# DerrickXuNu/CoBEVT

Measured on AMD Instinct MI355X. Metric: bev_frames_per_sec, higher is better.
Workload: dtype bf16

## Files before the change

cobevt_amd/csrc/basicblock.hip:

```cpp
#include "common.hpp"

namespace cobevt {

struct BasicBlockParams {
    const void* in;
    const uint4* w1;
    const float* b1;
    const uint4* w2;
    const float* b2;
    void* out;
    int N, H, W;
    int tiles_y, tiles_x;
    int ntiles;
};

#ifndef COBEVT_BB_PERSIST
#define COBEVT_BB_PERSIST 1
#endif

template <typename T, int C, int TH_> struct BBCfg {
    static constexpr int NT = 512;
    static constexpr int EB = Elem<T>::kBytes, CH = Elem<T>::kChunk;
    static constexpr int CC = 128 / EB;
    static constexpr int NCH = C / CC;
    static constexpr int NCT = C / 32;
    static constexpr int NPG = 8 / NCT;
    static constexpr int TH = TH_, TW = 16;
    static constexpr int R1H = TH + 2, R1W = TW + 2, R1 = R1H * R1W;
    static constexpr int N1 = (R1 + 31) / 32;
// ... 69 lines not shown
                    __builtin_amdgcn_sched_group_barrier(0x008, 1, 0);
                }
            }
            __builtin_amdgcn_sched_barrier(0);
        }
    }
}

#ifdef COBEVT_BB_TRACE
__device__ unsigned long long cobevt_bb_trace[32];
#define COBEVT_BB_MARK(i) do { if (blockIdx.x == 0 && threadIdx.x == 0) cobevt_bb_trace[(i)] = __builtin_readcyclecounter(); } while (0)
#else
#define COBEVT_BB_MARK(i) do {} while (0)
#endif

template <typename T, int C, int TH_>
__global__ __launch_bounds__(512, (C == 64 && TH_ == 8 && Elem<T>::kIsBf16) ? 4 : (TH_ == 12 ? 1 : 2)) void basicblock_kernel(BasicBlockParams p) {
    using G = BBCfg<T, C, TH_>;
    constexpr int NT = G::NT, CH = G::CH, CC = G::CC, NCH = G::NCH, NCT = G::NCT, NPG = G::NPG;
    constexpr int TH = G::TH, TW = G::TW, R1W = G::R1W, R1 = G::R1, N1 = G::N1, T1W = G::T1W, T2W = G::T2W;
    constexpr int P1W = G::P1W, PSTR1 = G::PSTR1, PSTR2 = G::PSTR2;
    constexpr int PIECES = 8;
    constexpr int P1_ITEMS = G::P1H * P1W * PIECES;
    constexpr int P_IT = (P1_ITEMS + NT - 1) / NT;
    constexpr int NSTEP = NCH * 9;
    constexpr int R = 3;

    extern __shared__ __attribute__((aligned(16))) unsigned char smem[];
    unsigned char* patch1 = smem;
    unsigned char* patch2 = smem + G::PATCH1;

    int logical;
// ... 135 lines not shown
                unsigned char* d = patch2 + ry * G::PITCH2 + rx * PSTR2 + (c0 + 8 * k) * Elem<T>::kBytes;
                if constexpr (Elem<T>::kIsBf16) *(uint2*)d = make_uint2(pack_bf2(v[0], v[1]), pack_bf2(v[2], v[3]));
                else if constexpr (kXPack<T, 4>)
                    *(uint2*)(patch2 + ry * G::PITCH2 + rx * PSTR2 + ct * 128 + packed_piece_offset(2 * k + h)) = make_uint2(pack_h2(v[0], v[1]), pack_h2(v[2], v[3]));
                else if constexpr (kXPack3<T, 4>)
                    store_piece_packed3(patch2 + ry * G::PITCH2 + rx * PSTR2 + ct * 128 + packed3_piece_offset(2 * k + h),
                                        make_uint4(__float_as_uint(v[0]), __float_as_uint(v[1]), __float_as_uint(v[2]), __float_as_uint(v[3])), false);
                else *(uint4*)d = stage_x_piece<T>(make_uint4(__float_as_uint(v[0]), __float_as_uint(v[1]), __float_as_uint(v[2]), __float_as_uint(v[3])));
            }
        }
    }
    constexpr int CPP = C / CH;
    constexpr int S_ITEMS = TH * TW * CPP;
    constexpr int S_IT = S_ITEMS / NT;
    static_assert(S_ITEMS % NT == 0, "store pass");
    int soff[S_IT];
    uint4 rres[S_IT];
#pragma unroll
    for (int i = 0; i < S_IT; ++i) {
        const int item = tid + i * NT;
        const int px = item / CPP, cj = item - px * CPP;
        const int oy = oy0 + px / TW, ox = ox0 + (px % TW);
        const bool ok = (oy < p.H) & (ox < p.W);
        soff[i] = ok ? ((img * p.H + oy) * p.W + ox) * C + cj * CH : -1;
        rres[i] = *(const uint4*)(in + (ok ? soff[i] : 0));
    }
    __builtin_amdgcn_sched_barrier(0);
    COBEVT_BB_MARK(8);
    __syncthreads();
    COBEVT_BB_MARK(9);

    f32x16 acc[T2W];
#pragma unroll
    for (int t = 0; t < T2W; ++t)
#pragma unroll
        for (int r = 0; r < 16; ++r) acc[t][r] = 0.f;
#pragma unroll 1
    for (int chunk = 0; chunk < NCH; ++chunk)
        bb_conv_chunk<T, T2W>(patch2 + chunk * 128, a2, t2_ok, G::PITCH2, PSTR2, w2src, chunk * 9, NSTEP, bq, acc);
    COBEVT_BB_MARK(10);
    const int next = tile + (int)gridDim.x;
    const bool has_next = G::PERSIST && next < p.ntiles;
    if (has_next) {
        set_tile(next);
        patch_addr();
        load_patch(0);
    }
    __syncthreads();
    COBEVT_BB_MARK(11);

    float* stage = (float*)smem;
    constexpr int SROW = G::SSTR / 4;
    {
        const int c0 = ct * 32 + 4 * h;
#pragma unroll
        for (int t = 0; t < T2W; ++t) {
            const int px = (pg + t * NPG) * 32 + ql;
#pragma unroll
            for (int k = 0; k < 4; ++k) {
                const float4 b = *(const float4*)&sbias[C + c0 + 8 * k];
                *(float4*)(stage + px * SROW + c0 + 8 * k) =
                    make_float4(acc[t][4 * k] + b.x, acc[t][4 * k + 1] + b.y, acc[t][4 * k + 2] + b.z, acc[t][4 * k + 3] + b.w);
            }
        }
    }
    __syncthreads();
    COBEVT_BB_MARK(12);
    T* out = (T*)p.out;
    float sv[S_IT][CH];
#pragma unroll
    for (int i = 0; i < S_IT; ++i) {
        const int item = tid + i * NT;
        const int px = item / CPP, cj = item - px * CPP;
#pragma unroll
        for (int e = 0; e < CH; ++e) sv[i][e] = stage[px * SROW + cj * CH + e];
    }
    if (has_next) __syncthreads();
#pragma unroll
    for (int i = 0; i < S_IT; ++i) {
        if (soff[i] < 0) continue;
        float v[8], rv[8];
#pragma unroll
        for (int e = 0; e < CH; ++e) v[e] = sv[i][e];
        chunk_to_f32<T>(rres[i], rv);
#pragma unroll
        for (int e = 0; e < CH; ++e) v[e] = fmaxf(v[e] + rv[e], 0.f);
        *(uint4*)(out + soff[i]) = f32_to_chunk<T>(v);
    }
    COBEVT_BB_MARK(13);
    if (!has_next) break;
    tile = next;
    load_b(bq[0], w1src, 0);
    load_b(bq[1], w1src, 1);
  }
}

template <typename T, int C, int TH_>
static int launch_basicblock(BasicBlockParams p, hipStream_t stream) {
    using G = BBCfg<T, C, TH_>;
    p.tiles_y = (p.H + G::TH - 1) / G::TH;
    p.tiles_x = (p.W + G::TW - 1) / G::TW;
    long blocks = (long)p.N * p.tiles_y * p.tiles_x;
    if (blocks <= 0 || blocks > 0x7fffffffL) return COBEVT_ERR_SHAPE;
    p.ntiles = (int)blocks;
    static cobevt::PerDeviceOnce attr_once;
    static int cu_slots[16];
    int dev = 0;
    (void)hipGetDevice(&dev);
    if (attr_once.first()) {
        (void)hipFuncSetAttribute((const void*)basicblock_kernel<T, C, TH_>, hipFuncAttributeMaxDynamicSharedMemorySize, G::LDS);
        int cus = 0;
        if (hipDeviceGetAttribute(&cus, hipDeviceAttributeMultiprocessorCount, dev) != hipSuccess || cus < 1) cus = 256;
        const int per_cu = (160 * 1024) / (G::LDS + 2048) < 1 ? 1 : (160 * 1024) / (G::LDS + 2048);
        cu_slots[dev & 15] = cus * (per_cu > 2 ? 2 : per_cu);
    }
    if (G::PERSIST && cu_slots[dev & 15] > 0 && blocks > cu_slots[dev & 15]) blocks = cu_slots[dev & 15];
    hipLaunchKernelGGL((basicblock_kernel<T, C, TH_>), dim3((unsigned)blocks), dim3(G::NT), G::LDS, stream, p);
    return hipGetLastError() == hipSuccess ? COBEVT_OK : COBEVT_ERR_LAUNCH;
}

struct DsBlockParams {
    const void* in;
    const uint4* w1;
    const float* b1;
    const uint4* w2;
    const float* b2;
    const uint4* wds;
    const float* bds;
    void* out;
    int N, H, W;
    int Ho, Wo;
    int tiles_y, tiles_x;
// ... 195 lines not shown
}

using namespace cobevt;

extern "C" int cobevt_basicblock_nhwc(const void* in, const void* wfrag1, const float* bias1, const void* wfrag2,
                                      const float* bias2, void* out, const int* dims, hipStream_t stream) {
    if (!in || !wfrag1 || !wfrag2 || !out || !dims) return COBEVT_ERR_ARG;
    BasicBlockParams p;
    p.in = in; p.w1 = (const uint4*)wfrag1; p.b1 = bias1; p.w2 = (const uint4*)wfrag2; p.b2 = bias2; p.out = out;
    const int dtype = dims[0];
    p.N = dims[1]; p.H = dims[2]; p.W = dims[3];
    const int c = dims[4];
    if (dtype != 0 && dtype != 1) return COBEVT_ERR_ARG;
    if (p.N < 1 || p.H < 1 || p.W < 1) return COBEVT_ERR_SHAPE;
    if ((long)p.N * p.H * p.W * c >= 0x7fffffffL) return COBEVT_ERR_UNSUPPORTED;
    const int th = dims[5];
    if (th != 0 && th != 8 && th != 12 && th != 16) return COBEVT_ERR_ARG;
    if (c == 128 && dtype == 0 && th == 12) return launch_basicblock<bf16_t, 128, 12>(p, stream);
    if (c == 64 && dtype == 0 && th == 8) return launch_basicblock<bf16_t, 64, 8>(p, stream);
    if (c == 64) return dtype == 0 ? launch_basicblock<bf16_t, 64, 16>(p, stream) : launch_basicblock<float, 64, 16>(p, stream);
    if (c == 128) return dtype == 0 ? launch_basicblock<bf16_t, 128, 8>(p, stream) : launch_basicblock<float, 128, 8>(p, stream);
    return COBEVT_ERR_UNSUPPORTED;
}

extern "C" int cobevt_dsblock_nhwc(const void* in, const void* wfrag1, const float* bias1, const void* wfrag2, const float* bias2,
                                   const void* wfrag_ds, const float* bias_ds, void* out, const int* dims, hipStream_t stream) {
    if (!in || !wfrag1 || !wfrag2 || !wfrag_ds || !out || !dims) return COBEVT_ERR_ARG;
    if (dims[0] != 0 || dims[4] != 64 || dims[5] != 128) return COBEVT_ERR_UNSUPPORTED;
    DsBlockParams p;
    p.in = in; p.w1 = (const uint4*)wfrag1; p.b1 = bias1; p.w2 = (const uint4*)wfrag2; p.b2 = bias2;
    p.wds = (const uint4*)wfrag_ds; p.bds = bias_ds; p.out = out;
    p.N = dims[1]; p.H = dims[2]; p.W = dims[3];
// ... 21 lines not shown
```

cobevt_amd/csrc/common.hpp:

```cpp
#pragma once
#include <hip/hip_runtime.h>
#include <stdint.h>

namespace cobevt {

struct bf16_t { uint16_t bits; };

using f32x4 = __attribute__((ext_vector_type(4))) float;
using f32x16 = __attribute__((ext_vector_type(16))) float;
using bf16x8 = __attribute__((ext_vector_type(8))) __bf16;

__device__ __forceinline__ float bf2f(uint16_t b) { return __uint_as_float(((uint32_t)b) << 16); }

using bf16x2 = __attribute__((ext_vector_type(2))) __bf16;
using f32x2 = __attribute__((ext_vector_type(2))) float;

__device__ __forceinline__ uint32_t pack_bf2(float lo, float hi) {
    const f32x2 v = {lo, hi};
    return __builtin_bit_cast(uint32_t, __builtin_convertvector(v, bf16x2));
}

__device__ __forceinline__ uint16_t f2bf(float f) { return (uint16_t)(pack_bf2(f, 0.f) & 0xffffu); }

template <typename T> struct Elem;
// ... 214 lines not shown
    split_bf16_pair(__uint_as_float(w0.x), __uint_as_float(w0.y), h[0], l[0]);
    split_bf16_pair(__uint_as_float(w0.z), __uint_as_float(w0.w), h[1], l[1]);
    split_bf16_pair(__uint_as_float(w1.x), __uint_as_float(w1.y), h[2], l[2]);
    split_bf16_pair(__uint_as_float(w1.z), __uint_as_float(w1.w), h[3], l[3]);
    wh = make_uint4(h[0], h[1], h[2], h[3]);
    wl = make_uint4(l[0], l[1], l[2], l[3]);
}
__device__ __forceinline__ void mfma_3term(const uint4& wh, const uint4& wl, const uint4& xh, const uint4& xl, f32x16& acc) {
    acc = __builtin_amdgcn_mfma_f32_32x32x16_bf16(__builtin_bit_cast(bf16x8, wh), __builtin_bit_cast(bf16x8, xh), acc, 0, 0, 0);
    acc = __builtin_amdgcn_mfma_f32_32x32x16_bf16(__builtin_bit_cast(bf16x8, wh), __builtin_bit_cast(bf16x8, xl), acc, 0, 0, 0);
    acc = __builtin_amdgcn_mfma_f32_32x32x16_bf16(__builtin_bit_cast(bf16x8, wl), __builtin_bit_cast(bf16x8, xh), acc, 0, 0, 0);
}

__device__ __forceinline__ int acc_row(int r, int lane) { return (r & 3) + 8 * (r >> 2) + 4 * (lane >> 5); }

__device__ __forceinline__ float erf_as(float x) {
    const float ax = fabsf(x);
    const float t = __builtin_amdgcn_rcpf(fmaf(0.3275911f, ax, 1.0f));
    float poly = fmaf(1.061405429f, t, -1.453152027f);
    poly = fmaf(poly, t, 1.421413741f);
    poly = fmaf(poly, t, -0.284496736f);
    poly = fmaf(poly, t, 0.254829592f);
    const float e = __builtin_amdgcn_exp2f(-ax * ax * 1.4426950408889634f);
    const float y = fmaf(-poly * t, e, 1.0f);
    return copysignf(y, x);
}

__device__ __forceinline__ float gelu_erf(float x) { return 0.5f * x * (1.0f + erf_as(x * 0.70710678118654752440f)); }

__device__ __forceinline__ float gelu_bf16(float x) {
// ... 49 lines not shown
```

cobevt_amd/csrc/conv3x3.hip:

```cpp
#include <type_traits>

#include "common.hpp"

namespace cobevt {

struct Conv3Params {
    const void* in;
    const void* wgt;
    const float* bias;
    const void* residual;
    void* out;
    int N, H, W, Cin;
    int Ho, Wo, Cout;
    int upsample;
    int act;
    int store_mode;
    int tiles_y, tiles_x, tiles_n;
    const void* in2 = nullptr;
    const float* bias2 = nullptr;
    int H2 = 0, W2 = 0, Cin2 = 0;
};

template <typename T, int NT, int NPX, int BN> struct Conv3Store {
    static constexpr int CH = Elem<T>::kChunk;
// ... 327 lines not shown
#define COBEVT_CONV3_CONT_LEAD 3
#endif
#ifndef COBEVT_CONV3_KNOCK
#define COBEVT_CONV3_KNOCK 0
#endif
#ifdef COBEVT_CONV3_TRACE
__device__ unsigned long long cobevt_conv3_trace[64];
__device__ unsigned long long cobevt_conv3_rt[3 * 2048];
#define COBEVT_TRACE_MARK(i) do { if (logical == 0 && tid == 0) cobevt_conv3_trace[(i)] = __builtin_readcyclecounter(); } while (0)
#define COBEVT_TRACE_RT(i) do { if (threadIdx.x == 0 && blockIdx.x < 2048) cobevt_conv3_rt[blockIdx.x * 3 + (i)] = (i) == 2 ? (unsigned long long)(__builtin_amdgcn_s_getreg((20 << 0) | (0 << 6) | (3 << 11)) & 15) : __builtin_amdgcn_s_memrealtime(); } while (0)
#else
#define COBEVT_TRACE_MARK(i) do {} while (0)
#define COBEVT_TRACE_RT(i) do {} while (0)
#endif

template <typename T, int MT, int WN, int KS, int S = 1, int NW = 8> struct Conv3SCfg {
    static constexpr int NT = 64 * NW, KG = 4, KGW = KG / KS;
    static constexpr bool HALF = NW == 4;
    static constexpr int BN = WN * 32;
    static constexpr int PW = S == 1 ? 18 : 33;
    static constexpr int SROWS = S == 1 ? 4 : 5;
    static constexpr int PSTR = KG * 32 + 16;
    static constexpr int PLANE = 17 * PSTR;
    static constexpr int PROW = ((S == 1 ? PW * PSTR : 2 * PLANE) + 255) / 256 * 256;
    static constexpr int STRIP_BYTES = SROWS * PROW;
    static constexpr int PATCH_BYTES = MT * STRIP_BYTES;
    static constexpr int SSTR = BN * 4 + 16;
    static constexpr int STAGE_BYTES = MT * 32 * SSTR;
    static constexpr int MAIN_BYTES = (S == 1 && !HALF ? 2 : 1) * PATCH_BYTES;
    static constexpr int LDS_BYTES = MAIN_BYTES > STAGE_BYTES ? MAIN_BYTES : STAGE_BYTES;
    static_assert(WN * KS == NW && (NW == 8 || (NW == 4 && S == 1)), "eight waves, or four (stride 1)");
};

template <typename T, int MT, int WN, int KS, int S, int NW, bool DS = false>
__global__ __launch_bounds__(64 * NW, NW == 4 ? 2 : 1) void conv3x3_strips_kernel(Conv3Params p) {
    static_assert(!DS || (Elem<T>::kIsBf16 && S == 1 && NW == 8), "the shortcut form is bf16 / stride 1 / eight waves");
    using C = Conv3SCfg<T, MT, WN, KS, S, NW>;
    constexpr bool HALF = C::HALF;
    constexpr int NT = C::NT, KG = C::KG, KGW = C::KGW, BN = C::BN, PW = C::PW;
    constexpr int CH = Elem<T>::kChunk;
    constexpr int CC = KG * 32 / Elem<T>::kBytes;
    constexpr int PSTR = C::PSTR, PROW = C::PROW, STRIP = C::STRIP_BYTES;
    constexpr int PIECES = 2 * KG;
    constexpr int STRIP_ITEMS = C::SROWS * PW * PIECES;
    constexpr int PATCH_ITEMS = MT * STRIP_ITEMS;
    constexpr int P_IT = S == 1 ? (PATCH_ITEMS + NT - 1) / NT : 1;
    constexpr int PF = 2, R = 3;
    constexpr bool PACK = kXPack<T, KGW>;
    constexpr bool PACK3 = kXPack3<T, KGW>;
    constexpr int KGA = (PACK || PACK3) ? KGW / 2 : KGW;
    constexpr int RA = PACK3 ? 2 : 3;
    constexpr bool CONT = COBEVT_CONV3_CONT && S == 1 && !HALF && Elem<T>::kIsBf16 && (KGA == 1 || KGA == 2) && MT <= 5;
// ... 170 lines not shown
            if (trace && r == 0) COBEVT_TRACE_MARK(58);
        }
    };
    if (S == 1) store_patch(patch);
    else fill_patch_s2(0);
    __syncthreads();
    COBEVT_TRACE_MARK(1);
    constexpr bool EARLY_RES = S == 1 && Elem<T>::kIsBf16 && MT <= 5;
    Conv3Store<T, NT, MT * 32, BN> st;
    auto coord = [&](int px, int& im, int& oy, int& ox) {
        const int4 sc = *(const int4*)&stab[(px >> 5) * 4];
        im = sc.x;
        oy = sc.y * 2 + ((px >> 4) & 1); ox = sc.z * 16 + (px & 15);
        return (sc.w != 0) & (oy < p.Ho) & (ox < p.Wo);
    };
    constexpr int PLT = (S == 1 && !HALF) ? (CONT ? PSF - COBEVT_CONV3_CONT_LEAD : COBEVT_CONV3_PLOAD_TAP) : 0;
    uint4 af[RA][MT];
    uint4 al[PACK3 ? RA : 1][PACK3 ? MT : 1];
    auto read_a_from = [&](const unsigned char* pb, int slot, int n) {
        const int t2 = n / KGA, g2 = n - t2 * KGA;
        const int kh2 = t2 / 3, kw2 = t2 - kh2 * 3;
        const int toff = S == 1 ? kh2 * PROW + kw2 * PSTR : kh2 * PROW + (kw2 & 1) * C::PLANE + (kw2 >> 1) * PSTR;
        const unsigned char* pn = pb + toff + abase + g2 * (PACK3 ? 64 : 32);
#pragma unroll
        for (int a = 0; a < MT; ++a) {
            af[slot][a] = *(const uint4*)(pn + a * STRIP);
            if constexpr (PACK3) al[slot][a] = *(const uint4*)(pn + a * STRIP + 16);
        }
    };
    if (CONT) {
// ... 16 lines not shown
        }
#pragma unroll
        for (int tap = 0; tap < 9; ++tap) {
            const int step = chunk * 9 + tap;
            if (chunk < 4) COBEVT_TRACE_MARK(2 + chunk * 9 + tap);
            if (CONT && tap == TB) {
                __syncthreads();
                __builtin_amdgcn_sched_barrier(0);
            }
#ifdef COBEVT_CONV3_SETPRIO
            if ((tap ^ ks) & 1) __builtin_amdgcn_s_setprio(3); else __builtin_amdgcn_s_setprio(0);
#endif
            if (!(COBEVT_CONV3_KNOCK & 1) || chunk == 0)
                load_b(bq[(tap + PF) % R], step + PF < nsteps ? step + PF : nsteps - 1);
            if (S == 1 && PLT > 0 && tap == PLT) {
                if (LAST) { if (EARLY_RES && p.store_mode == 0) st.prepare(p, tid, n0, coord); }
                else if (!(COBEVT_CONV3_KNOCK & 8)) load_patch(more ? chunk + 1 : chunk);
            }
            __builtin_amdgcn_sched_barrier(0);
#pragma unroll
            for (int g = 0; g < KGA; ++g) {
                const int n = tap * KGA + g;
                if (n + RA - 1 < NG) { if (!(COBEVT_CONV3_KNOCK & 4) || chunk == 0) read_a((n + RA - 1) % RA, n + RA - 1); }
                else if (CONT && !LAST && !(COBEVT_CONV3_KNOCK & 4)) read_a_from(pother, (n + RA - 1) % RA, n + RA - 1 - NG);
                uint4 wpk = make_uint4(0, 0, 0, 0), wlo = make_uint4(0, 0, 0, 0);
                if constexpr (PACK) wpk = pack_f16_pair(bq[tap % R][(2 * g) % KGW], bq[tap % R][(2 * g + 1) % KGW]);
                if constexpr (PACK3) split_w_pair(bq[tap % R][(2 * g) % KGW], bq[tap % R][(2 * g + 1) % KGW], wpk, wlo);
#pragma unroll
                for (int a = 0; a < MT; ++a) {
                    if (COBEVT_CONV3_KNOCK & 2) acc[a][0] += __uint_as_float((af[n % RA][a].x ^ bq[tap % R][g].x) & 0x3fffffffu);
                    else if constexpr (PACK) mfma_f16_packed(wpk, af[n % RA][a], acc[a]);
// ... 122 lines not shown
#pragma unroll
                for (int k = 0; k < 4; ++k) {
                    const uint32_t lo = pack_bf2(dacc[4 * k] + bias4[k].x, dacc[4 * k + 1] + bias4[k].y);
                    const uint32_t hi = pack_bf2(dacc[4 * k + 2] + bias4[k].z, dacc[4 * k + 3] + bias4[k].w);
                    acc[a][4 * k] += __uint_as_float(lo << 16);
                    acc[a][4 * k + 1] += __uint_as_float(lo & 0xffff0000u);
                    acc[a][4 * k + 2] += __uint_as_float(hi << 16);
                    acc[a][4 * k + 3] += __uint_as_float(hi & 0xffff0000u);
                }
            }
        }
        __syncthreads();
    }
    COBEVT_TRACE_MARK(38);

    reduce_ksplit(sbias, true);
    COBEVT_TRACE_MARK(39);
    T* out = (T*)p.out;
    if (p.store_mode == 0) {
        if (!EARLY_RES) st.prepare(p, tid, n0, coord);
        st.finish(p, stage, SROW, tid, n0);
    } else {
        const int cpp = BN * 4 / CH;
        for (int item = tid; item < MT * 8 * cpp; item += NT) {
            const int qp = item / cpp, cj = item - qp * cpp;
            const int s = qp >> 3, qx = qp & 7;
            const int4 sc = *(const int4*)&stab[s * 4];
            if (!sc.w) continue;
            const int img = sc.x, sy = sc.y, sx = sc.z;
            const int oy2 = sy, ox2 = sx * 8 + qx;
            if (oy2 >= (p.Ho >> 1) || ox2 >= (p.Wo >> 1)) continue;
            float v[8];
            bool any = false;
// ... 4 lines not shown
                float x = stage[px * SROW + c];
                x = p.act == 1 ? fmaxf(x, 0.f) : (p.act == 2 ? gelu_t<T>(x) : x);
                v[e] = x;
                any |= (n0 + c) < p.Cout;
            }
            if (!any) continue;
            const size_t o = (((size_t)img * (p.Ho >> 1) + oy2) * (p.Wo >> 1) + ox2) * (size_t)(p.Cout * 4) + (size_t)n0 * 4 + cj * CH;
            if (n0 + ((cj * CH + CH - 1) >> 2) < p.Cout && ((p.Cout * 4) % CH) == 0) *(uint4*)(out + o) = f32_to_chunk<T>(v);
            else for (int e = 0; e < CH; ++e) if (n0 + ((cj * CH + e) >> 2) < p.Cout) store_elem<T>(out, o + e, v[e]);
        }
    }
    COBEVT_TRACE_MARK(40);
    COBEVT_TRACE_RT(1);
}

template <typename T, int MT, int WN, int KS, int S, int NW = 8, bool DS = false>
static int launch_conv3s(Conv3Params p, int coutp, hipStream_t stream) {
    using C = Conv3SCfg<T, MT, WN, KS, S, NW>;
    if ((long)p.N * p.H * p.W * p.Cin >= 0x7fffffffL) return COBEVT_ERR_UNSUPPORTED;
    if (DS && (long)p.N * p.H2 * p.W2 * p.Cin2 >= 0x7fffffffL) return COBEVT_ERR_UNSUPPORTED;
    if (DS && (long)(p.Cin2 / 64) * MT * 32 * C::PSTR > (long)C::LDS_BYTES) return COBEVT_ERR_UNSUPPORTED;
    p.tiles_y = (p.Ho + 1) / 2;
    p.tiles_x = (p.Wo + 15) / 16;
    p.tiles_n = (p.Cout + C::BN - 1) / C::BN;
    if (p.tiles_n * C::BN > coutp) return COBEVT_ERR_SHAPE;
    const long nstrips = (long)p.N * p.tiles_y * p.tiles_x;
    const long blocks = (nstrips + MT - 1) / MT * p.tiles_n;
    if (blocks <= 0 || blocks > 0x7fffffffL) return COBEVT_ERR_SHAPE;
    constexpr size_t lds = C::LDS_BYTES;
    static cobevt::PerDeviceOnce attr_once;
    if (attr_once.first()) {
        (void)hipFuncSetAttribute((const void*)conv3x3_strips_kernel<T, MT, WN, KS, S, NW, DS>, hipFuncAttributeMaxDynamicSharedMemorySize, (int)lds);
    }
    hipLaunchKernelGGL((conv3x3_strips_kernel<T, MT, WN, KS, S, NW, DS>), dim3((unsigned)blocks), dim3(C::NT), lds, stream, p);
    return hipGetLastError() == hipSuccess ? COBEVT_OK : COBEVT_ERR_LAUNCH;
}

template <typename T, int MT>
static int launch_conv3s_bn(const Conv3Params& p, int coutp, int bn64, int stride, hipStream_t stream) {
    if constexpr (Elem<T>::kIsBf16 && MT <= 5) {
        if (bn64 == 3 && stride == 1) return launch_conv3s<T, MT, 1, 4, 1, 4>(p, coutp, stream);
    }
    if (bn64 > 1) return COBEVT_ERR_UNSUPPORTED;
    if (stride == 2) return bn64 ? launch_conv3s<T, MT, 2, 4, 2>(p, coutp, stream) : launch_conv3s<T, MT, 4, 2, 2>(p, coutp, stream);
    return bn64 ? launch_conv3s<T, MT, 2, 4, 1>(p, coutp, stream) : launch_conv3s<T, MT, 4, 2, 1>(p, coutp, stream);
}

template <typename T>
static int dispatch_conv3f(const Conv3Params& p, int kg, int coutp, int variant, int stride, hipStream_t stream) {
    if (kg != 4) return COBEVT_ERR_UNSUPPORTED;
    if (variant == 0) variant = p.Cout <= 64 ? 151 : 150;
    const int mt = (variant - 100) / 10, bn64 = (variant - 100) % 10;
    if (variant < 100 || bn64 > 3) return COBEVT_ERR_ARG;
    if constexpr (Elem<T>::kIsBf16) {
        if (bn64 == 3 && stride == 1 && mt == 1) return launch_conv3s<T, 1, 1, 4, 1, 4>(p, coutp, stream);
        if (bn64 == 3 && stride == 1 && mt == 2) return launch_conv3s<T, 2, 1, 4, 1, 4>(p, coutp, stream);
    }
    switch (mt) {
        case 3: return launch_conv3s_bn<T, 3>(p, coutp, bn64, stride, stream);
        case 4: return launch_conv3s_bn<T, 4>(p, coutp, bn64, stride, stream);
        case 5: return launch_conv3s_bn<T, 5>(p, coutp, bn64, stride, stream);
        case 6: return launch_conv3s_bn<T, 6>(p, coutp, bn64, stride, stream);
        default: return COBEVT_ERR_ARG;
    }
}

}

using namespace cobevt;

extern "C" int cobevt_conv3x3_nhwc(const void* in, const void* wgt, const float* bias, const void* residual, void* out,
                                   const int* dims, hipStream_t stream) {
    if (!in || !wgt || !out || !dims) return COBEVT_ERR_ARG;
    Conv3Params p;
    const int dtype = dims[0];
    p.in = in; p.wgt = wgt; p.bias = bias; p.residual = residual; p.out = out;
    p.N = dims[1]; p.H = dims[2]; p.W = dims[3]; p.Cin = dims[4]; p.Cout = dims[5];
// ... 37 lines not shown
    if (p.store_mode == 1 && (p.residual || ((p.Ho | p.Wo) & 1))) return COBEVT_ERR_UNSUPPORTED;
    if (p.Cin % cc != 0 || coutp % 32 != 0 || coutp < p.Cout) return COBEVT_ERR_SHAPE;
    const int kg = cc * (dtype == 0 ? 2 : 4) / 32;
    return dtype == 0 ? dispatch_conv3f<bf16_t>(p, kg, coutp, variant, stride, stream)
                      : dispatch_conv3f<float>(p, kg, coutp, variant, stride, stream);
}

extern "C" int cobevt_conv3x3_ds_wfrag_nhwc(const void* in, const void* in2, const void* wfrag, const float* bias, const float* bias2, void* out,
                                            const int* dims, hipStream_t stream) {
    if (!in || !in2 || !wfrag || !out || !dims) return COBEVT_ERR_ARG;
    if (dims[0] != 0) return COBEVT_ERR_UNSUPPORTED;
    Conv3Params p;
    p.in = in; p.wgt = wfrag; p.bias = bias; p.bias2 = bias2; p.residual = nullptr; p.out = out; p.in2 = in2;
    p.N = dims[1]; p.H = dims[2]; p.W = dims[3]; p.Cin = dims[4]; p.Cout = dims[5];
    p.upsample = 0; p.act = dims[6]; p.store_mode = 0;
    const int coutp = dims[7], variant = dims[8];
    p.H2 = dims[9]; p.W2 = dims[10]; p.Cin2 = dims[11];
    p.Ho = p.H; p.Wo = p.W;
    if (p.N < 1 || p.H < 1 || p.W < 1 || p.Cin < 64 || p.Cin % 64 || p.Cout < 1 || p.Cin2 < 64 || p.Cin2 % 64) return COBEVT_ERR_SHAPE;
    if (p.Cin2 > 256) return COBEVT_ERR_UNSUPPORTED;
    if ((p.H2 - 1) / 2 + 1 != p.H || (p.W2 - 1) / 2 + 1 != p.W) return COBEVT_ERR_SHAPE;
    if (coutp % 32 != 0 || coutp < p.Cout) return COBEVT_ERR_SHAPE;
    if (p.act < 0 || p.act > 2) return COBEVT_ERR_ARG;
    const int mt = (variant - 100) / 10, bn64 = (variant - 100) % 10;
    if (variant < 100 || bn64 > 1) return COBEVT_ERR_ARG;
    switch (mt * 2 + bn64) {
        case 6: return launch_conv3s<bf16_t, 3, 4, 2, 1, 8, true>(p, coutp, stream);
        case 7: return launch_conv3s<bf16_t, 3, 2, 4, 1, 8, true>(p, coutp, stream);
        case 8: return launch_conv3s<bf16_t, 4, 4, 2, 1, 8, true>(p, coutp, stream);
        case 9: return launch_conv3s<bf16_t, 4, 2, 4, 1, 8, true>(p, coutp, stream);
        case 10: return launch_conv3s<bf16_t, 5, 4, 2, 1, 8, true>(p, coutp, stream);
        case 11: return launch_conv3s<bf16_t, 5, 2, 4, 1, 8, true>(p, coutp, stream);
        default: return COBEVT_ERR_UNSUPPORTED;
    }
}

#ifdef COBEVT_CONV3_TRACE
extern "C" int cobevt_conv3_read_trace(unsigned long long* dst) {
    return hipMemcpyFromSymbol(dst, HIP_SYMBOL(cobevt_conv3_trace), sizeof(unsigned long long) * 64) == hipSuccess ? 0 : 1;
}
extern "C" int cobevt_conv3_read_rt(unsigned long long* dst) {
    return hipMemcpyFromSymbol(dst, HIP_SYMBOL(cobevt_conv3_rt), sizeof(unsigned long long) * 3 * 2048) == hipSuccess ? 0 : 1;
}
#endif
```

cobevt_amd/ops.py:

```python
import ctypes
import os
import math

import torch

from . import lib as _L
from .lib import CobevtHipError

BF16, FP32 = 0, 1
USE_CONV3X3 = True
USE_CONV3_S2 = True
USE_CONV3_SMALL_TILES = True
USE_CONV3_DS = True
USE_CONV3_WFRAG = True
CONV3_VARIANT = 0
USE_GEMM_ROWS = True
USE_GEMM_ROWS2 = False
USE_GEMM_ROWS3 = True
GEMM_ROWS3_MIN_M = 0
GEMM_ROWS3_MAX_K = 512
GEMM_ROWS3_STRIDED = 1
GEMM_ROWS3_ROWS64_MIN_M = 0
USE_STEM_POOL = True
USE_STEM = True
ROW_CHAIN_ROWS = 0
USE_ROW_CHAIN = True
USE_BOTTLENECK_F32 = True
USE_GEMM_ROWS3_F32 = True
USE_ROW_CHAIN_F32 = True
BASICBLOCK_TILE_ROWS = 0
USE_BASICBLOCK = True
BASICBLOCK_MAX_C = 128
USE_DSBLOCK = True
USE_EMBED_GEMM = False
USE_EMBED_GEMM3 = True
USE_CHAIN_NEXT = True
USE_HEAD_CONV = True
USE_PROJ_CHAIN = True
USE_PROJ_CHAIN_KV = True
USE_PROJ_CHAIN_WAVE = True
USE_SWAP_STAGE = True
USE_BOTTLENECK = True
ATTN_VARIANT = 0
USE_ATTN_BIG_RESIDENT = False
ATTN_KSPLIT = 2
ATTN_QSPLIT = 0

# ... 354 lines not shown
                                                        ctypes.c_float(plan.ln_eps), _stream())
            else:
                rc = _L.load().cobevt_linear_rows(_p(x), _p(plan.wgt_rows), _p(plan.bias), _p(residual), None, None,
                                                  _p(plan.pre_scale), _p(plan.pre_shift), _p(out), ldims,
                                                  ctypes.c_float(plan.ln_eps), _stream())
        _L.check(rc, "cobevt_linear_rows_wfrag" if v2 else "cobevt_linear_rows")
        return out
    variant = 0
    if plan.wfrag is not None and (out_h, out_w) == (ho, wo) and USE_CONV3X3 and USE_CONV3_WFRAG \
            and (plan.stride == 1 or (USE_CONV3_S2 and not (plan.code == FP32 and _L.get_variant() == "f32s"))):
        variant = CONV3_VARIANT or conv3_tiling(n, ho, wo, cin, plan.cout, plan.cc3, stride=plan.stride, bf16=plan.code == BF16,
                                                packed=(0.5 if _L.get_variant() == "f32h" else 0.75 if _L.get_variant() == "f32s" else 0) if plan.code == FP32 else 0)
        if variant == 0 and plan.stride == 2:
            variant = 151 if plan.cout <= 64 else 150
    if variant > 0:
        dims = _ints([plan.code, n, h, w, cin, plan.cout, plan.upsample, plan.act, sm, plan.cc3, plan.coutp3, variant,
                      plan.stride])
        with _timed("conv3x3|%d->%d %dx%dx%d" % (cin, plan.cout, n, ho, wo), cost):
            rc = _L.load().cobevt_conv3x3_wfrag_nhwc(_p(x), _p(plan.wfrag), _p(plan.bias), _p(residual), _p(out), dims, _stream())
        _L.check(rc, "cobevt_conv3x3_wfrag_nhwc")
        return out
    if plan.wgt3 is not None and (out_h, out_w) == (ho, wo) and USE_CONV3X3:
        dims = _ints([plan.code, n, h, w, cin, plan.cout, plan.upsample, plan.act, sm, plan.cc3])
        with _timed("conv3x3|%d->%d %dx%dx%d" % (cin, plan.cout, n, ho, wo), cost):
            rc = _L.load().cobevt_conv3x3_nhwc(_p(x), _p(plan.wgt3), _p(plan.bias), _p(residual), _p(out), dims, _stream())
        _L.check(rc, "cobevt_conv3x3_nhwc")
        return out
    dims = _ints([plan.code, n, h, w, cin, ho, wo, plan.cout, plan.kh, plan.kw, plan.stride, plan.pad, plan.K,
                  plan.kpad, plan.upsample, plan.pre_relu, plan.act, sm, out_h, out_w, plan.smallc])
    with _timed("igemm|k%ds%d %d->%d M=%d%s" % (plan.kh, plan.stride, cin, plan.cout, n * ho * wo, " stem" if plan.smallc else ""), cost):
        rc = _L.load().cobevt_conv2d_nhwc(_p(x), _p(plan.wgt), _p(plan.bias), _p(residual), _p(plan.pre_scale),
                                          _p(plan.pre_shift), _p(plan.klut), _p(out), dims, _stream())
    _L.check(rc, "cobevt_conv2d_nhwc")
    return out


def basicblock_fusable(x, plan1, plan2):
    return (USE_BASICBLOCK and plan1.wfrag is not None and plan2.wfrag is not None and plan1.cin == plan1.cout == plan2.cin
            == plan2.cout and plan1.cout in (64, 128) and plan1.cout <= BASICBLOCK_MAX_C and plan1.act == 1 and plan2.act == 1 and not plan1.upsample
            and not plan2.upsample and plan1.store_mode == 0 and plan2.store_mode == 0 and x.is_contiguous()
            and x.dtype == plan1.dtype and x.numel() < 2 ** 31)


def basicblock(x, plan1, plan2):
    _need_cuda(x)
    n, h, w, c = x.shape
    out = torch.empty_like(x)
    dims = _ints([plan1.code, n, h, w, c, BASICBLOCK_TILE_ROWS])

    def cost():
        esz = 2 if plan1.code == BF16 else 4
        return 2.0 * 2 * n * h * w * c * 9 * c, float(2 * x.numel() * esz + 2 * c * 9 * c * esz)

    with _timed("basicblock|%d %dx%dx%d" % (c, n, h, w), cost):
        rc = _L.load().cobevt_basicblock_nhwc(_p(x), _p(plan1.wfrag), _p(plan1.bias), _p(plan2.wfrag), _p(plan2.bias),
                                              _p(out), dims, _stream())
    _L.check(rc, "cobevt_basicblock_nhwc")
    return out


def dsblock_fusable(x, plan1, plan2, plan_ds):
    return (USE_DSBLOCK and x.dtype == torch.bfloat16 and plan1.dtype == torch.bfloat16 and x.dim() == 4 and x.is_contiguous()
            and plan1.wfrag is not None and plan2.wfrag is not None and plan_ds.wfrag_rows is not None
# ... 46 lines not shown
    main = plan2.wfrag.reshape(t, (cin // 64) * 9, 2048)
    wd = torch.zeros((coutp, cin2), dtype=plan2.wfrag.dtype, device=plan2.wfrag.device)
    wd[:plan_ds.cout] = plan_ds.wgt_rows[:, :cin2]
    extra = wd.reshape(t, 32, cin2 // 64, 4, 2, 8).permute(0, 2, 3, 4, 1, 5).reshape(t, cin2 // 64, 2048)
    table = torch.cat([main, extra], dim=1).contiguous()
    plan2._ds_fused = (plan_ds, table)
    return table


def conv3_ds(y, x, plan2, plan_ds, variant):
    _need_cuda(y, x)
    n, ho, wo, c = y.shape
    _, h, w, cin2 = x.shape
    table = _conv3_ds_table(plan2, plan_ds)
    out = torch.empty((n, ho, wo, plan2.cout), dtype=y.dtype, device=y.device)
    dims = _ints([plan2.code, n, ho, wo, c, plan2.cout, plan2.act, plan2.coutp3, variant, h, w, cin2])

    def cost():
        px = n * ho * wo
        return 2.0 * px * plan2.cout * (9 * c + cin2), float(2 * (y.numel() + px * cin2 + out.numel()) + 2 * plan2.cout * (9 * c + cin2))

    with _timed("conv3x3|%d->%d +ds%d %dx%dx%d" % (c, plan2.cout, cin2, n, ho, wo), cost):
        rc = _L.load().cobevt_conv3x3_ds_wfrag_nhwc(_p(y), _p(x), _p(table), _p(plan2.bias), _p(plan_ds.bias), _p(out), dims, _stream())
    _L.check(rc, "cobevt_conv3x3_ds_wfrag_nhwc")
    return out


class BottleneckPlan(object):

    def __init__(self, conv1, bn1, conv2, bn2, conv3, bn3, device="cuda"):
        def fold(conv, bn):
# ... 896 lines not shown
```

Baseline: 613.1.

## Store conv epilogues directly from MFMA registers using permlane32 swaps

Adds a bf16 register epilogue to the fused basic block and the strip conv3x3 kernels. Accumulators get bias, residual and activation applied in registers and are written to global memory directly, using permlane32_swap to pair output-channel runs into contiguous 16-byte stores. The basic block drops the LDS staging round trip and its barriers. In the conv3x3 kernel the k-split partial sums are still exchanged through a smaller LDS buffer, but each owning wave reduces and stores its own rows. The new path is the default, with a flag bit to fall back to the staged path; the cost is more register pressure and narrower store patterns per lane.

```diff
diff --git a/cobevt_amd/csrc/basicblock.hip b/cobevt_amd/csrc/basicblock.hip
--- a/cobevt_amd/csrc/basicblock.hip
+++ b/cobevt_amd/csrc/basicblock.hip
@@ -13,6 +13,7 @@
     int tiles_y, tiles_x;
     int ntiles;
 };
+
 
 #ifndef COBEVT_BB_PERSIST
 #define COBEVT_BB_PERSIST 1
@@ -112,8 +113,9 @@
 #define COBEVT_BB_MARK(i) do {} while (0)
 #endif
 
-template <typename T, int C, int TH_>
+template <typename T, int C, int TH_, bool REG = false>
 __global__ __launch_bounds__(512, (C == 64 && TH_ == 8 && Elem<T>::kIsBf16) ? 4 : (TH_ == 12 ? 1 : 2)) void basicblock_kernel(BasicBlockParams p) {
+    static_assert(!REG || Elem<T>::kIsBf16, "the register epilogue is bf16 only");
     using G = BBCfg<T, C, TH_>;
     constexpr int NT = G::NT, CH = G::CH, CC = G::CC, NCH = G::NCH, NCT = G::NCT, NPG = G::NPG;
     constexpr int TH = G::TH, TW = G::TW, R1W = G::R1W, R1 = G::R1, N1 = G::N1, T1W = G::T1W, T2W = G::T2W;
@@ -279,16 +281,30 @@
     constexpr int S_ITEMS = TH * TW * CPP;
     constexpr int S_IT = S_ITEMS / NT;
     static_assert(S_ITEMS % NT == 0, "store pass");
-    int soff[S_IT];
-    uint4 rres[S_IT];
-#pragma unroll
-    for (int i = 0; i < S_IT; ++i) {
-        const int item = tid + i * NT;
-        const int px = item / CPP, cj = item - px * CPP;
-        const int oy = oy0 + px / TW, ox = ox0 + (px % TW);
-        const bool ok = (oy < p.H) & (ox < p.W);
-        soff[i] = ok ? ((img * p.H + oy) * p.W + ox) * C + cj * CH : -1;
-        rres[i] = *(const uint4*)(in + (ok ? soff[i] : 0));
+    int soff[REG ? 1 : S_IT];
+    uint4 rres[REG ? 1 : S_IT];
+    int eoff[REG ? T2W : 1];
+    uint4 eres[REG ? T2W : 1][2];
+    if constexpr (REG) {
+#pragma unroll
+        for (int t = 0; t < T2W; ++t) {
+            const int px = (pg + t * NPG) * 32 + ql;
+            const int oy = oy0 + px / TW, ox = ox0 + (px % TW);
+            const bool ok = (oy < p.H) & (ox < p.W);
+            eoff[t] = ok ? ((img * p.H + oy) * p.W + ox) * C + ct * 32 + 8 * h : -1;
+#pragma unroll
+            for (int m = 0; m < 2; ++m) eres[t][m] = *(const uint4*)(in + (ok ? eoff[t] + 16 * m : 0));
+        }
+    } else {
+#pragma unroll
+        for (int i = 0; i < S_IT; ++i) {
+            const int item = tid + i * NT;
+            const int px = item / CPP, cj = item - px * CPP;
+            const int oy = oy0 + px / TW, ox = ox0 + (px % TW);
+            const bool ok = (oy < p.H) & (ox < p.W);
+            soff[i] = ok ? ((img * p.H + oy) * p.W + ox) * C + cj * CH : -1;
+            rres[i] = *(const uint4*)(in + (ok ? soff[i] : 0));
+        }
     }
     __builtin_amdgcn_sched_barrier(0);
     COBEVT_BB_MARK(8);
@@ -311,6 +327,27 @@
         patch_addr();
         load_patch(0);
     }
+    T* out = (T*)p.out;
+    if constexpr (REG) {
+        COBEVT_BB_MARK(11);
+        COBEVT_BB_MARK(12);
+#pragma unroll
+        for (int t = 0; t < T2W; ++t) {
+#pragma unroll
+            for (int m = 0; m < 2; ++m) {
+                const float4 b0 = *(const float4*)&sbias[C + ct * 32 + 16 * m + 4 * h];
+                const float4 b1v = *(const float4*)&sbias[C + ct * 32 + 16 * m + 8 + 4 * h];
+                float v[8] = {acc[t][8 * m] + b0.x, acc[t][8 * m + 1] + b0.y, acc[t][8 * m + 2] + b0.z, acc[t][8 * m + 3] + b0.w,
+                              acc[t][8 * m + 4] + b1v.x, acc[t][8 * m + 5] + b1v.y, acc[t][8 * m + 6] + b1v.z, acc[t][8 * m + 7] + b1v.w};
+                float rv[8];
+                unpair_cout_runs(eres[t][m], rv);
+#pragma unroll
+                for (int e = 0; e < 8; ++e) v[e] = fmaxf(v[e] + rv[e], 0.f);
+                const uint4 piece = pair_cout_runs(pack_bf2(v[0], v[1]), pack_bf2(v[2], v[3]), pack_bf2(v[4], v[5]), pack_bf2(v[6], v[7]));
+                if (eoff[t] >= 0) *(uint4*)(out + eoff[t] + 16 * m) = piece;
+            }
+        }
+    } else {
     __syncthreads();
     COBEVT_BB_MARK(11);
 
@@ -331,7 +368,6 @@
     }
     __syncthreads();
     COBEVT_BB_MARK(12);
-    T* out = (T*)p.out;
     float sv[S_IT][CH];
 #pragma unroll
     for (int i = 0; i < S_IT; ++i) {
@@ -351,6 +387,7 @@
 #pragma unroll
         for (int e = 0; e < CH; ++e) v[e] = fmaxf(v[e] + rv[e], 0.f);
         *(uint4*)(out + soff[i]) = f32_to_chunk<T>(v);
+    }
     }
     COBEVT_BB_MARK(13);
     if (!has_next) break;
@@ -360,7 +397,7 @@
   }
 }
 
-template <typename T, int C, int TH_>
+template <typename T, int C, int TH_, bool REG = false>
 static int launch_basicblock(BasicBlockParams p, hipStream_t stream) {
     using G = BBCfg<T, C, TH_>;
     p.tiles_y = (p.H + G::TH - 1) / G::TH;
@@ -373,14 +410,14 @@
     int dev = 0;
     (void)hipGetDevice(&dev);
     if (attr_once.first()) {
-        (void)hipFuncSetAttribute((const void*)basicblock_kernel<T, C, TH_>, hipFuncAttributeMaxDynamicSharedMemorySize, G::LDS);
+        (void)hipFuncSetAttribute((const void*)basicblock_kernel<T, C, TH_, REG>, hipFuncAttributeMaxDynamicSharedMemorySize, G::LDS);
         int cus = 0;
         if (hipDeviceGetAttribute(&cus, hipDeviceAttributeMultiprocessorCount, dev) != hipSuccess || cus < 1) cus = 256;
         const int per_cu = (160 * 1024) / (G::LDS + 2048) < 1 ? 1 : (160 * 1024) / (G::LDS + 2048);
         cu_slots[dev & 15] = cus * (per_cu > 2 ? 2 : per_cu);
     }
     if (G::PERSIST && cu_slots[dev & 15] > 0 && blocks > cu_slots[dev & 15]) blocks = cu_slots[dev & 15];
-    hipLaunchKernelGGL((basicblock_kernel<T, C, TH_>), dim3((unsigned)blocks), dim3(G::NT), G::LDS, stream, p);
+    hipLaunchKernelGGL((basicblock_kernel<T, C, TH_, REG>), dim3((unsigned)blocks), dim3(G::NT), G::LDS, stream, p);
     return hipGetLastError() == hipSuccess ? COBEVT_OK : COBEVT_ERR_LAUNCH;
 }
 
@@ -606,8 +643,17 @@
     if (dtype != 0 && dtype != 1) return COBEVT_ERR_ARG;
     if (p.N < 1 || p.H < 1 || p.W < 1) return COBEVT_ERR_SHAPE;
     if ((long)p.N * p.H * p.W * c >= 0x7fffffffL) return COBEVT_ERR_UNSUPPORTED;
-    const int th = dims[5];
+    const int th = dims[5] & 0x3ff;
+    const bool staged = (dims[5] & 0x400) != 0;
+    if (dims[5] & ~0x7ff) return COBEVT_ERR_ARG;
     if (th != 0 && th != 8 && th != 12 && th != 16) return COBEVT_ERR_ARG;
+    if (dtype == 0 && !staged) {
+        if (c == 128 && th == 12) return launch_basicblock<bf16_t, 128, 12, true>(p, stream);
+        if (c == 64 && th == 8) return launch_basicblock<bf16_t, 64, 8, true>(p, stream);
+        if (c == 64) return launch_basicblock<bf16_t, 64, 16, true>(p, stream);
+        if (c == 128) return launch_basicblock<bf16_t, 128, 8, true>(p, stream);
+        return COBEVT_ERR_UNSUPPORTED;
+    }
     if (c == 128 && dtype == 0 && th == 12) return launch_basicblock<bf16_t, 128, 12>(p, stream);
     if (c == 64 && dtype == 0 && th == 8) return launch_basicblock<bf16_t, 64, 8>(p, stream);
     if (c == 64) return dtype == 0 ? launch_basicblock<bf16_t, 64, 16>(p, stream) : launch_basicblock<float, 64, 16>(p, stream);
diff --git a/cobevt_amd/csrc/common.hpp b/cobevt_amd/csrc/common.hpp
--- a/cobevt_amd/csrc/common.hpp
+++ b/cobevt_amd/csrc/common.hpp
@@ -252,6 +252,20 @@
 
 __device__ __forceinline__ int acc_row(int r, int lane) { return (r & 3) + 8 * (r >> 2) + 4 * (lane >> 5); }
 
+__device__ __forceinline__ uint4 pair_cout_runs(uint32_t r0x, uint32_t r0y, uint32_t r1x, uint32_t r1y) {
+    const auto sx = __builtin_amdgcn_permlane32_swap(r0x, r1x, false, false);
+    const auto sy = __builtin_amdgcn_permlane32_swap(r0y, r1y, false, false);
+    return make_uint4(sx[0], sy[0], sx[1], sy[1]);
+}
+__device__ __forceinline__ void unpair_cout_runs(const uint4& piece, float (&rv)[8]) {
+    const auto sx = __builtin_amdgcn_permlane32_swap(piece.x, piece.z, false, false);
+    const auto sy = __builtin_amdgcn_permlane32_swap(piece.y, piece.w, false, false);
+    rv[0] = __uint_as_float(sx[0] << 16); rv[1] = __uint_as_float(sx[0] & 0xffff0000u);
+    rv[2] = __uint_as_float(sy[0] << 16); rv[3] = __uint_as_float(sy[0] & 0xffff0000u);
+    rv[4] = __uint_as_float(sx[1] << 16); rv[5] = __uint_as_float(sx[1] & 0xffff0000u);
+    rv[6] = __uint_as_float(sy[1] << 16); rv[7] = __uint_as_float(sy[1] & 0xffff0000u);
+}
+
 __device__ __forceinline__ float erf_as(float x) {
     const float ax = fabsf(x);
     const float t = __builtin_amdgcn_rcpf(fmaf(0.3275911f, ax, 1.0f));
diff --git a/cobevt_amd/csrc/conv3x3.hip b/cobevt_amd/csrc/conv3x3.hip
--- a/cobevt_amd/csrc/conv3x3.hip
+++ b/cobevt_amd/csrc/conv3x3.hip
@@ -365,7 +365,7 @@
 #define COBEVT_TRACE_RT(i) do {} while (0)
 #endif
 
-template <typename T, int MT, int WN, int KS, int S = 1, int NW = 8> struct Conv3SCfg {
+template <typename T, int MT, int WN, int KS, int S = 1, int NW = 8, bool REG = false> struct Conv3SCfg {
     static constexpr int NT = 64 * NW, KG = 4, KGW = KG / KS;
     static constexpr bool HALF = NW == 4;
     static constexpr int BN = WN * 32;
@@ -379,14 +379,16 @@
     static constexpr int SSTR = BN * 4 + 16;
     static constexpr int STAGE_BYTES = MT * 32 * SSTR;
     static constexpr int MAIN_BYTES = (S == 1 && !HALF ? 2 : 1) * PATCH_BYTES;
-    static constexpr int LDS_BYTES = MAIN_BYTES > STAGE_BYTES ? MAIN_BYTES : STAGE_BYTES;
+    static constexpr int XCH_BYTES = REG ? MT * WN * (KS - 1) * 4096 : 0;
+    static constexpr int LDS_BYTES = (MAIN_BYTES > STAGE_BYTES ? MAIN_BYTES : STAGE_BYTES) > XCH_BYTES ? (MAIN_BYTES > STAGE_BYTES ? MAIN_BYTES : STAGE_BYTES) : XCH_BYTES;
     static_assert(WN * KS == NW && (NW == 8 || (NW == 4 && S == 1)), "eight waves, or four (stride 1)");
 };
 
-template <typename T, int MT, int WN, int KS, int S, int NW, bool DS = false>
+template <typename T, int MT, int WN, int KS, int S, int NW, bool DS = false, bool REG = false>
 __global__ __launch_bounds__(64 * NW, NW == 4 ? 2 : 1) void conv3x3_strips_kernel(Conv3Params p) {
     static_assert(!DS || (Elem<T>::kIsBf16 && S == 1 && NW == 8), "the shortcut form is bf16 / stride 1 / eight waves");
-    using C = Conv3SCfg<T, MT, WN, KS, S, NW>;
+    static_assert(!REG || (Elem<T>::kIsBf16 && NW == 8 && (KS & (KS - 1)) == 0), "the register epilogue is bf16 / eight waves");
+    using C = Conv3SCfg<T, MT, WN, KS, S, NW, REG>;
     constexpr bool HALF = C::HALF;
     constexpr int NT = C::NT, KG = C::KG, KGW = C::KGW, BN = C::BN, PW = C::PW;
     constexpr int CH = Elem<T>::kChunk;
@@ -587,6 +589,27 @@
         oy = sc.y * 2 + ((px >> 4) & 1); ox = sc.z * 16 + (px & 15);
         return (sc.w != 0) & (oy < p.Ho) & (ox < p.Wo);
     };
+    constexpr int NOWN = (MT + KS - 1) / KS;
+    long eoff[REG ? NOWN : 1];
+    uint4 eres[REG ? NOWN : 1][2];
+    auto reg_prepare = [&](int ks_, int wn_, int h_, int ql_) {
+        if constexpr (REG) {
+#pragma unroll
+            for (int j = 0; j < NOWN; ++j) {
+                const int a = ((ks_ + KS - 1) & (KS - 1)) + j * KS;
+                int im, oy, ox;
+                const bool ok = coord((a < MT ? a : 0) * 32 + ql_, im, oy, ox) & (a < MT);
+                eoff[j] = ok ? (((long)im * p.Ho + oy) * p.Wo + ox) * p.Cout + n0 + wn_ * 32 + 8 * h_ : -1;
+                eres[j][0] = eres[j][1] = make_uint4(0, 0, 0, 0);
+            }
+            if (p.residual) {
+#pragma unroll
+                for (int j = 0; j < NOWN; ++j)
+#pragma unroll
+                    for (int m = 0; m < 2; ++m) eres[j][m] = *(const uint4*)((const T*)p.residual + (eoff[j] < 0 ? 0 : eoff[j] + 16 * m));
+            }
+        }
+    };
     constexpr int PLT = (S == 1 && !HALF) ? (CONT ? PSF - COBEVT_CONV3_CONT_LEAD : COBEVT_CONV3_PLOAD_TAP) : 0;
     uint4 af[RA][MT];
     uint4 al[PACK3 ? RA : 1][PACK3 ? MT : 1];
@@ -633,7 +656,10 @@
             if (!(COBEVT_CONV3_KNOCK & 1) || chunk == 0)
                 load_b(bq[(tap + PF) % R], step + PF < nsteps ? step + PF : nsteps - 1);
             if (S == 1 && PLT > 0 && tap == PLT) {
-                if (LAST) { if (EARLY_RES && p.store_mode == 0) st.prepare(p, tid, n0, coord); }
+                if (LAST) {
+                    if constexpr (REG) { if (EARLY_RES) reg_prepare(ks, wn, h, ql); }
+                    else if (EARLY_RES && p.store_mode == 0) st.prepare(p, tid, n0, coord);
+                }
                 else if (!(COBEVT_CONV3_KNOCK & 8)) load_patch(more ? chunk + 1 : chunk);
             }
             __builtin_amdgcn_sched_barrier(0);
@@ -786,9 +812,73 @@
     }
     COBEVT_TRACE_MARK(38);
 
+    T* out = (T*)p.out;
+    if constexpr (REG) {
+        int te = threadIdx.x;
+        asm volatile("" : "+v"(te));
+        const int lanee = te & 63, he = lanee >> 5, wne = (te >> 6) % WN, kse = (te >> 6) / WN;
+        const int xlane = wne * ((KS - 1) * 256) + lanee;
+        const int c0 = wne * 32 + 4 * he;
+        float4 bias4[4];
+#pragma unroll
+        for (int k = 0; k < 4; ++k) bias4[k] = *(const float4*)&sbias[c0 + 8 * k];
+        COBEVT_TRACE_MARK(57);
+        float4* xch = (float4*)smem + xlane;
+#pragma unroll
+        for (int a = 0; a < MT; ++a) {
+            if (((a + 1) & (KS - 1)) == kse) continue;
+            const int r = (a - kse) & (KS - 1);
+            float4* xw = xch + (a * WN * (KS - 1) + r) * 256;
+#pragma unroll
+            for (int k = 0; k < 4; ++k) {
+                float4 v = make_float4(acc[a][4 * k], acc[a][4 * k + 1], acc[a][4 * k + 2], acc[a][4 * k + 3]);
+                if (r == 0) { v.x += bias4[k].x; v.y += bias4[k].y; v.z += bias4[k].z; v.w += bias4[k].w; }
+                xw[k * 64] = v;
+            }
+        }
+        if (!EARLY_RES) reg_prepare(kse, wne, he, lanee & 31);
+        __syncthreads();
+        COBEVT_TRACE_MARK(58);
+        COBEVT_TRACE_MARK(39);
+#pragma unroll
+        for (int a = 0; a < MT; ++a) {
+            if (((a + 1) & (KS - 1)) != kse) continue;
+            const int j = a / KS;
+            const float4* xr = xch + a * WN * (KS - 1) * 256;
+            float4 part[KS - 1][4];
+#pragma unroll
+            for (int r = 0; r < KS - 1; ++r)
+#pragma unroll
+                for (int k = 0; k < 4; ++k) part[r][k] = xr[r * 256 + k * 64];
+#pragma unroll
+            for (int m = 0; m < 2; ++m) {
+                float v[8];
+#pragma unroll
+                for (int e = 0; e < 8; ++e) {
+                    const int k = 2 * m + (e >> 2), c = e & 3;
+                    float sum = c == 0 ? part[0][k].x : c == 1 ? part[0][k].y : c == 2 ? part[0][k].z : part[0][k].w;
+#pragma unroll
+                    for (int r = 1; r < KS - 1; ++r) sum += c == 0 ? part[r][k].x : c == 1 ? part[r][k].y : c == 2 ? part[r][k].z : part[r][k].w;
+                    v[e] = sum + acc[a][4 * k + c];
+                }
+                if (p.residual) {
+                    float rv[8];
+                    unpair_cout_runs(eres[j][m], rv);
+#pragma unroll
+                    for (int e = 0; e < 8; ++e) v[e] += rv[e];
+                }
+#pragma unroll
+                for (int e = 0; e < 8; ++e) v[e] = p.act == 1 ? fmaxf(v[e], 0.f) : (p.act == 2 ? gelu_t<T>(v[e]) : v[e]);
+                const uint4 piece = pair_cout_runs(pack_bf2(v[0], v[1]), pack_bf2(v[2], v[3]), pack_bf2(v[4], v[5]), pack_bf2(v[6], v[7]));
+                if (eoff[j] >= 0) *(uint4*)(out + eoff[j] + 16 * m) = piece;
+            }
+        }
+        COBEVT_TRACE_MARK(40);
+        COBEVT_TRACE_RT(1);
+        return;
+    }
     reduce_ksplit(sbias, true);
     COBEVT_TRACE_MARK(39);
-    T* out = (T*)p.out;
     if (p.store_mode == 0) {
         if (!EARLY_RES) st.prepare(p, tid, n0, coord);
         st.finish(p, stage, SROW, tid, n0);
@@ -823,9 +913,9 @@
     COBEVT_TRACE_RT(1);
 }
 
-template <typename T, int MT, int WN, int KS, int S, int NW = 8, bool DS = false>
+template <typename T, int MT, int WN, int KS, int S, int NW = 8, bool DS = false, bool REG = false>
 static int launch_conv3s(Conv3Params p, int coutp, hipStream_t stream) {
-    using C = Conv3SCfg<T, MT, WN, KS, S, NW>;
+    using C = Conv3SCfg<T, MT, WN, KS, S, NW, REG>;
     if ((long)p.N * p.H * p.W * p.Cin >= 0x7fffffffL) return COBEVT_ERR_UNSUPPORTED;
     if (DS && (long)p.N * p.H2 * p.W2 * p.Cin2 >= 0x7fffffffL) return COBEVT_ERR_UNSUPPORTED;
     if (DS && (long)(p.Cin2 / 64) * MT * 32 * C::PSTR > (long)C::LDS_BYTES) return COBEVT_ERR_UNSUPPORTED;
@@ -839,25 +929,36 @@
     constexpr size_t lds = C::LDS_BYTES;
     static cobevt::PerDeviceOnce attr_once;
     if (attr_once.first()) {
-        (void)hipFuncSetAttribute((const void*)conv3x3_strips_kernel<T, MT, WN, KS, S, NW, DS>, hipFuncAttributeMaxDynamicSharedMemorySize, (int)lds);
-    }
-    hipLaunchKernelGGL((conv3x3_strips_kernel<T, MT, WN, KS, S, NW, DS>), dim3((unsigned)blocks), dim3(C::NT), lds, stream, p);
+        (void)hipFuncSetAttribute((const void*)conv3x3_strips_kernel<T, MT, WN, KS, S, NW, DS, REG>, hipFuncAttributeMaxDynamicSharedMemorySize, (int)lds);
+    }
+    hipLaunchKernelGGL((conv3x3_strips_kernel<T, MT, WN, KS, S, NW, DS, REG>), dim3((unsigned)blocks), dim3(C::NT), lds, stream, p);
     return hipGetLastError() == hipSuccess ? COBEVT_OK : COBEVT_ERR_LAUNCH;
 }
 
+template <typename T, int MT, int WN, int KS, int S, bool DS = false>
+static int launch_conv3s_epi(const Conv3Params& p, int coutp, bool staged, hipStream_t stream) {
+    constexpr bool kRegFits = !(S == 2 && (MT == 6 || (MT == 5 && WN == 4)));
+    if constexpr (Elem<T>::kIsBf16 && kRegFits) {
+        if (!staged && p.store_mode == 0 && p.Cout % (WN * 32) == 0) return launch_conv3s<T, MT, WN, KS, S, 8, DS, true>(p, coutp, stream);
+    }
+    return launch_conv3s<T, MT, WN, KS, S, 8, DS>(p, coutp, stream);
+}
+
 template <typename T, int MT>
-static int launch_conv3s_bn(const Conv3Params& p, int coutp, int bn64, int stride, hipStream_t stream) {
+static int launch_conv3s_bn(const Conv3Params& p, int coutp, int bn64, int stride, bool staged, hipStream_t stream) {
     if constexpr (Elem<T>::kIsBf16 && MT <= 5) {
         if (bn64 == 3 && stride == 1) return launch_conv3s<T, MT, 1, 4, 1, 4>(p, coutp, stream);
     }
     if (bn64 > 1) return COBEVT_ERR_UNSUPPORTED;
-    if (stride == 2) return bn64 ? launch_conv3s<T, MT, 2, 4, 2>(p, coutp, stream) : launch_conv3s<T, MT, 4, 2, 2>(p, coutp, stream);
-    return bn64 ? launch_conv3s<T, MT, 2, 4, 1>(p, coutp, stream) : launch_conv3s<T, MT, 4, 2, 1>(p, coutp, stream);
+    if (stride == 2) return bn64 ? launch_conv3s_epi<T, MT, 2, 4, 2>(p, coutp, staged, stream) : launch_conv3s_epi<T, MT, 4, 2, 2>(p, coutp, staged, stream);
+    return bn64 ? launch_conv3s_epi<T, MT, 2, 4, 1>(p, coutp, staged, stream) : launch_conv3s_epi<T, MT, 4, 2, 1>(p, coutp, staged, stream);
 }
 
 template <typename T>
 static int dispatch_conv3f(const Conv3Params& p, int kg, int coutp, int variant, int stride, hipStream_t stream) {
     if (kg != 4) return COBEVT_ERR_UNSUPPORTED;
+    const bool staged = (variant & 0x400) != 0;
+    variant &= ~0x400;
     if (variant == 0) variant = p.Cout <= 64 ? 151 : 150;
     const int mt = (variant - 100) / 10, bn64 = (variant - 100) % 10;
     if (variant < 100 || bn64 > 3) return COBEVT_ERR_ARG;
@@ -866,10 +967,10 @@
         if (bn64 == 3 && stride == 1 && mt == 2) return launch_conv3s<T, 2, 1, 4, 1, 4>(p, coutp, stream);
     }
     switch (mt) {
-        case 3: return launch_conv3s_bn<T, 3>(p, coutp, bn64, stride, stream);
-        case 4: return launch_conv3s_bn<T, 4>(p, coutp, bn64, stride, stream);
-        case 5: return launch_conv3s_bn<T, 5>(p, coutp, bn64, stride, stream);
-        case 6: return launch_conv3s_bn<T, 6>(p, coutp, bn64, stride, stream);
+        case 3: return launch_conv3s_bn<T, 3>(p, coutp, bn64, stride, staged, stream);
+        case 4: return launch_conv3s_bn<T, 4>(p, coutp, bn64, stride, staged, stream);
+        case 5: return launch_conv3s_bn<T, 5>(p, coutp, bn64, stride, staged, stream);
+        case 6: return launch_conv3s_bn<T, 6>(p, coutp, bn64, stride, staged, stream);
         default: return COBEVT_ERR_ARG;
     }
 }
@@ -937,7 +1038,8 @@
     p.in = in; p.wgt = wfrag; p.bias = bias; p.bias2 = bias2; p.residual = nullptr; p.out = out; p.in2 = in2;
     p.N = dims[1]; p.H = dims[2]; p.W = dims[3]; p.Cin = dims[4]; p.Cout = dims[5];
     p.upsample = 0; p.act = dims[6]; p.store_mode = 0;
-    const int coutp = dims[7], variant = dims[8];
+    const int coutp = dims[7], variant = dims[8] & ~0x400;
+    const bool staged = (dims[8] & 0x400) != 0;
     p.H2 = dims[9]; p.W2 = dims[10]; p.Cin2 = dims[11];
     p.Ho = p.H; p.Wo = p.W;
     if (p.N < 1 || p.H < 1 || p.W < 1 || p.Cin < 64 || p.Cin % 64 || p.Cout < 1 || p.Cin2 < 64 || p.Cin2 % 64) return COBEVT_ERR_SHAPE;
@@ -948,12 +1050,12 @@
     const int mt = (variant - 100) / 10, bn64 = (variant - 100) % 10;
     if (variant < 100 || bn64 > 1) return COBEVT_ERR_ARG;
     switch (mt * 2 + bn64) {
-        case 6: return launch_conv3s<bf16_t, 3, 4, 2, 1, 8, true>(p, coutp, stream);
-        case 7: return launch_conv3s<bf16_t, 3, 2, 4, 1, 8, true>(p, coutp, stream);
-        case 8: return launch_conv3s<bf16_t, 4, 4, 2, 1, 8, true>(p, coutp, stream);
-        case 9: return launch_conv3s<bf16_t, 4, 2, 4, 1, 8, true>(p, coutp, stream);
-        case 10: return launch_conv3s<bf16_t, 5, 4, 2, 1, 8, true>(p, coutp, stream);
-        case 11: return launch_conv3s<bf16_t, 5, 2, 4, 1, 8, true>(p, coutp, stream);
+        case 6: return launch_conv3s_epi<bf16_t, 3, 4, 2, 1, true>(p, coutp, staged, stream);
+        case 7: return launch_conv3s_epi<bf16_t, 3, 2, 4, 1, true>(p, coutp, staged, stream);
+        case 8: return launch_conv3s_epi<bf16_t, 4, 4, 2, 1, true>(p, coutp, staged, stream);
+        case 9: return launch_conv3s_epi<bf16_t, 4, 2, 4, 1, true>(p, coutp, staged, stream);
+        case 10: return launch_conv3s_epi<bf16_t, 5, 4, 2, 1, true>(p, coutp, staged, stream);
+        case 11: return launch_conv3s_epi<bf16_t, 5, 2, 4, 1, true>(p, coutp, staged, stream);
         default: return COBEVT_ERR_UNSUPPORTED;
     }
 }
diff --git a/cobevt_amd/ops.py b/cobevt_amd/ops.py
--- a/cobevt_amd/ops.py
+++ b/cobevt_amd/ops.py
@@ -31,6 +31,7 @@
 BASICBLOCK_TILE_ROWS = 0
 USE_BASICBLOCK = True
 BASICBLOCK_MAX_C = 128
+USE_REG_EPILOGUE = True
 USE_DSBLOCK = True
 USE_EMBED_GEMM = False
 USE_EMBED_GEMM3 = True
@@ -415,7 +416,7 @@
         if variant == 0 and plan.stride == 2:
             variant = 151 if plan.cout <= 64 else 150
     if variant > 0:
-        dims = _ints([plan.code, n, h, w, cin, plan.cout, plan.upsample, plan.act, sm, plan.cc3, plan.coutp3, variant,
+        dims = _ints([plan.code, n, h, w, cin, plan.cout, plan.upsample, plan.act, sm, plan.cc3, plan.coutp3, variant | _epilogue_bit(),
                       plan.stride])
         with _timed("conv3x3|%d->%d %dx%dx%d" % (cin, plan.cout, n, ho, wo), cost):
             rc = _L.load().cobevt_conv3x3_wfrag_nhwc(_p(x), _p(plan.wfrag), _p(plan.bias), _p(residual), _p(out), dims, _stream())
@@ -436,6 +437,13 @@
     return out
 
 
+STAGED_EPILOGUE_BIT = 0x400
+
+
+def _epilogue_bit():
+    return 0 if USE_REG_EPILOGUE else STAGED_EPILOGUE_BIT
+
+
 def basicblock_fusable(x, plan1, plan2):
     return (USE_BASICBLOCK and plan1.wfrag is not None and plan2.wfrag is not None and plan1.cin == plan1.cout == plan2.cin
             == plan2.cout and plan1.cout in (64, 128) and plan1.cout <= BASICBLOCK_MAX_C and plan1.act == 1 and plan2.act == 1 and not plan1.upsample
@@ -447,7 +455,7 @@
     _need_cuda(x)
     n, h, w, c = x.shape
     out = torch.empty_like(x)
-    dims = _ints([plan1.code, n, h, w, c, BASICBLOCK_TILE_ROWS])
+    dims = _ints([plan1.code, n, h, w, c, BASICBLOCK_TILE_ROWS | _epilogue_bit()])
 
     def cost():
         esz = 2 if plan1.code == BF16 else 4
@@ -524,7 +532,7 @@
     _, h, w, cin2 = x.shape
     table = _conv3_ds_table(plan2, plan_ds)
     out = torch.empty((n, ho, wo, plan2.cout), dtype=y.dtype, device=y.device)
-    dims = _ints([plan2.code, n, ho, wo, c, plan2.cout, plan2.act, plan2.coutp3, variant, h, w, cin2])
+    dims = _ints([plan2.code, n, ho, wo, c, plan2.cout, plan2.act, plan2.coutp3, variant | _epilogue_bit(), h, w, cin2])
 
     def cost():
         px = n * ho * wo
```

Measured after the change: 618.2 (median of 6 runs). Within noise of the previous version (+0.8%).
